# yzhang1918/www2023tiger

Hardware: NVIDIA B200
Metric: events/sec (memory update + embedding, batch 200) (higher is better)
Workload: dtype f32

## Files before the change

include/tiger_b200.h:

```cpp
#ifndef TIGER_B200_H
#define TIGER_B200_H

#include <stdint.h>

#ifdef __cplusplus
extern "C" {
#endif

#define TIGER_OK 0
#define TIGER_EINVAL (-1)
#define TIGER_ECUDA (-2)

#define TIGER_ERR_PAST_MEMORY 1u
#define TIGER_ERR_UNUSED_MSG 2u
#define TIGER_ERR_MSG_BEFORE_MEM 4u
#define TIGER_ERR_MSG_TS_MISMATCH 8u
#define TIGER_ERR_EVENT_BEFORE_MEM 16u
#define TIGER_ERR_CAPACITY 32u

int tiger_abi_version(void);


int64_t tiger_csr_build_work_bytes(int64_t n_events, int64_t n_nodes);
int tiger_csr_build(const int64_t* src, const int64_t* dst, const double* ts, const int64_t* eid,
// ... 9 lines not shown
int tiger_hit_window(const int64_t* center, const int64_t* neigh, int64_t n, int k, float* hit,
                     void* stream);

int tiger_mark_nodes(const int64_t* ids, int64_t n, uint32_t* bitmap, int64_t n_nodes, void* stream);

int tiger_compact_involved(uint32_t* bitmap, int64_t n_nodes, uint8_t* has_msg, uint8_t* uptodate,
                           int64_t* involved, int64_t cap_involved, int64_t* local_index,
                           int64_t* outdated, int32_t* gru_row, int64_t* restart_nodes,
                           int32_t* counts, uint32_t* err_flags, void* stream);


int tiger_select_latest(const int64_t* nids, const void* ts, int ts_is_f64, int64_t n,
                        int64_t ts_period, int64_t n_nodes, uint64_t* slot_ts, uint32_t* slot_pos, uint32_t* bitmap,
                        uint8_t* winner, int64_t* unique_ids, int64_t* index, int32_t* count,
                        void* stream);

int tiger_anonymized_reindex(const int64_t* hist_nids, int64_t n, int len, int64_t* out,
                             const int32_t* count, void* stream);


int tiger_gather_rows(const float* table, int64_t width, const int64_t* ids, int64_t n, float* out,
                      const float* ts_table, float* out_ts, void* stream);

int tiger_scatter_rows(float* table, int64_t width, const int64_t* ids, int64_t n,
                       const int32_t* count, const float* vals, float* ts_table, const float* ts,
                       uint8_t* active, int check, uint32_t* err_flags, void* stream);

int tiger_time_encode(const float* ts, int64_t n, const float* w, const float* b, int dim, float* out,
                      void* stream);

// ... 155 lines not shown
                                  int64_t m_rows, int k_dim, const tiger_left_writeback_fused* wb, void* stream);

int tiger_sgemm_nt_packed_splitk_fused(const float* A, int64_t lda, const float* wpack, int bn, const float* bias,
                                       float* C, int64_t ldc, int k_parts, int64_t m_rows, const int32_t* count,
                                       int64_t rows_per_count, int n_cols, int k_dim, float alpha, int relu,
                                       void* stream);

void* tiger_pipe_create(int n_slots);
void tiger_pipe_destroy(void* pipe);
int tiger_pipe_capture_begin(void* stream);
int tiger_pipe_capture_end(void* pipe, void* stream, int slot, int kind);
int tiger_pipe_submit(void* pipe, int slot, const void* src, void* d_in, int64_t in_bytes, const void* d_out, void* h_out,
                      int64_t out_bytes, void* main_stream);
int tiger_pipe_wait(void* pipe, int slot, int host_results);
int tiger_pipe_join(void* pipe, void* stream);


int tiger_train_gather_pending(const int64_t* ids, const int32_t* count, int64_t cap, const float* msg_vals, int m_dim, const float* msg_ts, const float* upd_vals, int d, const float* check_mem_ts, int check_equal, float* X, float* H, float* dh_zero, uint32_t* err_flags, float* n_rows_out, void* stream);
int tiger_train_gru_gates(const float* Gi, const float* Gh, const float* H, const int32_t* count, int64_t cap, int d, float* h_new, float* r_out, float* z_out, float* n_out, void* stream);
int tiger_train_gru_gates_bwd(const float* dh, const float* r_in, const float* z_in, const float* n_in, const float* Gh, const float* H, const int32_t* count, int64_t cap, int d, float* dGi, float* dGh, void* stream);
int tiger_train_attn_build_ex(const int64_t* center, int64_t n_q, const float* ts, int64_t batch, int64_t ts_group, const int64_t* neigh_nids, const int64_t* neigh_eids, const float* neigh_ts, int k, const float* rows_a, const float* rows_b, const float* key_rows, const int32_t* sel, const float* nfeats, const float* efeats, int d, int de, const float* time_w, const float* time_b, float* q_in, float* kv_in, float* cat, int64_t ld_cat, int cat_off, void* stream);
int tiger_train_attn_core(const float* Q, int64_t ldq, const float* Kp, const float* Vp, int64_t ldkv, const int64_t* neigh_nids, int64_t n_q, int k, int n_head, int head_dim, float p_drop, int seed, float* attn, int64_t ld_attn, float* P, uint32_t* keep_bits, uint8_t* empty, void* stream);
int tiger_train_attn_core_bwd(const float* dattn, int64_t ld_attn, const float* Q, int64_t ldq, const float* Kp, const float* Vp, int64_t ldkv, const float* P, const uint32_t* keep_bits, int64_t n_q, int k, int n_head, int head_dim, float p_drop, float* dQ, float* dKp, float* dVp, void* stream);
int tiger_train_attn_build_bwd_ex(const float* dkv_in, const float* dq_in, const float* dcat, int64_t ld_cat, int cat_off, const int64_t* center, int64_t n_q, const float* ts, int64_t batch, int64_t ts_group, const int64_t* neigh_nids, const float* neigh_ts, int k, const int32_t* sel, int d, int de, const float* time_w, const float* time_b, float* dh_new, float* d_key_rows, float* g_time_w, float* g_time_b, void* stream);
int tiger_train_zero_rows(float* buf, int64_t ld, int cols, int64_t n_rows, const uint8_t* flag, void* stream);
int tiger_train_relu_bwd(float* dy, int64_t ld_dy, const float* y, int64_t ld_y, int cols, int64_t n_rows, const int32_t* count, int64_t rows_per_count, float scale, void* stream);
int tiger_train_colsum(const float* X, int64_t ld, int64_t n_rows, const int32_t* count, int64_t rows_per_count, int cols, float scale, float* out, void* stream);
int tiger_train_scatter_add_rows(float* table, const int64_t* ids, int64_t n, const int32_t* count, int64_t rows_per_count, const float* src, int64_t ld_src, int width, float scale, void* stream);
int tiger_train_score_build(const float* z, const float* hits, const int64_t* neigh_nids, const int64_t* batch_nids, int k, const float* hit_emb, int64_t batch, int d, float* pair, uint8_t* codes, void* stream);
int tiger_train_score_head(float* hid, const float* fc2_w, const float* fc2_b, int64_t batch, int d, float p_drop, int seed, float* scores, float* loss, float* dscore, void* stream);
// ... 27 lines not shown
```

www2023tiger_b200/_lib.py:

```python
import ctypes
import os
import re
from typing import Dict, List

import torch

from .build import INCLUDE, LIB_PATH

P, L, I, F = ctypes.c_void_p, ctypes.c_int64, ctypes.c_int, ctypes.c_float

_SIGNATURES: Dict[str, str] = {
    'tiger_abi_version': '',
    'tiger_csr_build_work_bytes': 'll',
    'tiger_csr_build': 'ppppll' + 'ppppp' + 'p' + 'p',
    'tiger_find_recent': 'ppppp' + 'pp' + 'lli' + 'pppp' + 'pp' + 'p' + 'p',
    'tiger_hit_window': 'ppli' + 'p' + 'p',
    'tiger_mark_nodes': 'plpl' + 'p',
    'tiger_compact_involved': 'plpp' + 'plp' + 'ppp' + 'pp' + 'p',
    'tiger_select_latest': 'ppil' + 'llppp' + 'pppp' + 'p',
    'tiger_anonymized_reindex': 'plip' + 'p' + 'p',
    'tiger_gather_rows': 'plplp' + 'pp' + 'p',
    'tiger_scatter_rows': 'plplp' + 'ppp' + 'pip' + 'p',
    'tiger_time_encode': 'plppip' + 'p',
    'tiger_store_messages': 'ppppl' + 'ppp' + 'ppii' + 'pppp' + 'pp' + 'p',
    'tiger_store_messages_dense': 'ppppl' + 'p' + 'pppp' + 'ppii' + 'pppp' + 'pp' + 'p',
    'tiger_right_writeback': 'plp' + 'ppi' + 'pppp' + 'pppp' + 'p' + 'p',
    'tiger_left_writeback': 'pllp' + 'pip' + 'ppp' + 'p' + 'p',
    'tiger_gru_pack_bytes': 'ii',
    'tiger_gru_pack': 'ppiip' + 'p',
    'tiger_gru_update': 'ppl' + 'plpl' + 'ii' + 'p' + 'ppp' + 'ppi' + 'p' + 'p',
    'tiger_gru_update_rows': 'ppl' + 'plpl' + 'ii' + 'p' + 'ppp' + 'ppi' + 'p' + 'p',
    'tiger_merge_pack': 'piipp',
    'tiger_merge_update': 'ppl' + 'plipl' + 'ii' + 'ppp' + 'ppi' + 'p' + 'p',
    'tiger_attn_fold_bytes': 'iii',
    'tiger_attn_fold': 'piii' + 'p',
    'tiger_temporal_attention_work_bytes': 'liiii',
    'tiger_temporal_attention_ex': 'pplll' + 'pppi' + 'ppppi' + 'pp' + 'iii' + 'ppp' + 'p',
    'tiger_temporal_attention_dense': 'pppppp' + 'li' + 'iii' + 'ppp' + 'p',
    'tiger_score_fold_bytes': 'i',
    'tiger_score_fold_cab_offset': 'i',
    'tiger_score_fold': 'pppppip' + 'p',
    'tiger_link_score_folded': 'pli' + 'pppp' + 'i' + 'ppp' + 'ppp' + 'p',
    'tiger_sgemm_nt_packed_gather': 'ppi' + 'pplp' + 'pi' + 'ppl' + 'lpl' + 'iifi' + 'p',
    'tiger_sgemm_nt_packed_splitk_fused': 'plpi' + 'ppl' + 'i' + 'lpl' + 'iifi' + 'p',
    'tiger_pipe_capture_begin': 'p',
    'tiger_pipe_capture_end': 'ppii',
    'tiger_pipe_submit': 'pipplpplp',
    'tiger_pipe_wait': 'pii',
    'tiger_pipe_join': 'pp',
    'tiger_sgemm_nt_packed_scatter': 'plpippli' + 'pliil' + 'ip' + 'p',
    'tiger_min_time': 'plp' + 'p',
    'tiger_seq_tokens': 'ppli' + 'ppppp' + 'ppii' + 'ppp' + 'ppp' + 'p',
    'tiger_sgemm_nt': 'plplp' + 'pl' + 'lpl' + 'iii' + 'p',
    'tiger_train_gather_pending': 'pplpippipipppppp',
    'tiger_train_gru_gates': 'pppplippppp',
    'tiger_train_gru_gates_bwd': 'ppppppplippp',
    'tiger_train_attn_build_ex': 'plpll' + 'pppi' + 'ppppp' + 'p' + 'ii' + 'pp' + 'ppp' + 'li' + 'p',
    'tiger_train_attn_core': 'plpplpliiifiplpppp',
    'tiger_train_attn_core_bwd': 'plplpplppliiifpppp',
    'tiger_train_attn_build_bwd_ex': 'pppli' + 'plpll' + 'ppi' + 'pii' + 'pp' + 'pppp' + 'p',
    'tiger_train_zero_rows': 'plilpp',
    'tiger_train_relu_bwd': 'plplilplfp',
    'tiger_train_colsum': 'pllplifpp',
    'tiger_train_scatter_add_rows': 'pplplplifp',
# ... 101 lines not shown
```

www2023tiger_b200/csrc/pipe.cu:

```cuda
#include <vector>

#include "common.cuh"

struct TigerPipe {
  int n_slots;
  cudaStream_t s_in, s_out;
  std::vector<cudaGraphExec_t> finder, model, tail;
  std::vector<cudaEvent_t> ev_in, ev_done, ev_out;
  std::vector<char> used, has_out;
  int last_slot;
};

extern "C" void* tiger_pipe_create(int n_slots) {
  if (n_slots <= 0 || n_slots > 1024) return nullptr;
  TigerPipe* p = new TigerPipe();
  p->n_slots = n_slots;
  if (cudaStreamCreateWithFlags(&p->s_in, cudaStreamNonBlocking) != cudaSuccess ||
      cudaStreamCreateWithFlags(&p->s_out, cudaStreamNonBlocking) != cudaSuccess) {
    delete p;
    return nullptr;
  }
  p->finder.assign(n_slots, nullptr);
  p->model.assign(n_slots, nullptr);
  p->tail.assign(n_slots, nullptr);
  p->has_out.assign(n_slots, 0);
  p->last_slot = -1;
  p->ev_in.resize(n_slots);
  p->ev_done.resize(n_slots);
  p->ev_out.resize(n_slots);
  p->used.assign(n_slots, 0);
  for (int i = 0; i < n_slots; ++i) {
    cudaEventCreateWithFlags(&p->ev_in[i], cudaEventDisableTiming);
    cudaEventCreateWithFlags(&p->ev_done[i], cudaEventDisableTiming);
    cudaEventCreateWithFlags(&p->ev_out[i], cudaEventDisableTiming);
  }
  return p;
}

extern "C" void tiger_pipe_destroy(void* pipe) {
  TigerPipe* p = reinterpret_cast<TigerPipe*>(pipe);
  if (p == nullptr) return;
  for (int i = 0; i < p->n_slots; ++i) {
    if (p->finder[i] != nullptr) cudaGraphExecDestroy(p->finder[i]);
    if (p->model[i] != nullptr) cudaGraphExecDestroy(p->model[i]);
    if (p->tail[i] != nullptr) cudaGraphExecDestroy(p->tail[i]);
    cudaEventDestroy(p->ev_in[i]);
    cudaEventDestroy(p->ev_done[i]);
    cudaEventDestroy(p->ev_out[i]);
  }
  cudaStreamDestroy(p->s_in);
  cudaStreamDestroy(p->s_out);
  delete p;
}

extern "C" int tiger_pipe_capture_begin(void* stream) {
  return cudaStreamBeginCapture(as_stream(stream), cudaStreamCaptureModeRelaxed) == cudaSuccess ? TIGER_OK : TIGER_ECUDA;
}

extern "C" int tiger_pipe_capture_end(void* pipe, void* stream, int slot, int kind) {
  TigerPipe* p = reinterpret_cast<TigerPipe*>(pipe);
  cudaGraph_t graph = nullptr;
  if (cudaStreamEndCapture(as_stream(stream), &graph) != cudaSuccess || graph == nullptr) return TIGER_ECUDA;
  if (p == nullptr || slot < 0 || slot >= p->n_slots || kind < 0 || kind > 2) {
    cudaGraphDestroy(graph);
    return TIGER_EINVAL;
  }
  cudaGraphExec_t exec = nullptr;
  const cudaError_t err = cudaGraphInstantiate(&exec, graph, 0);
  cudaGraphDestroy(graph);
  if (err != cudaSuccess) return TIGER_ECUDA;
  cudaGraphExec_t& dst = kind == 0 ? p->finder[slot] : (kind == 1 ? p->model[slot] : p->tail[slot]);
  if (dst != nullptr) cudaGraphExecDestroy(dst);
  dst = exec;
  return TIGER_OK;
}

extern "C" int tiger_pipe_submit(void* pipe, int slot, const void* src, void* d_in, int64_t in_bytes, const void* d_out,
                                 void* h_out, int64_t out_bytes, void* main_stream) {
  TigerPipe* p = reinterpret_cast<TigerPipe*>(pipe);
  if (p == nullptr || slot < 0 || slot >= p->n_slots || p->finder[slot] == nullptr || p->model[slot] == nullptr ||
      src == nullptr || d_in == nullptr || in_bytes <= 0)
    return TIGER_EINVAL;
  cudaStream_t main = as_stream(main_stream);
  bool ok = true;
  if (p->used[slot])
    ok = ok && cudaStreamWaitEvent(p->s_in, p->has_out[slot] ? p->ev_out[slot] : p->ev_done[slot], 0) == cudaSuccess;
  ok = ok && cudaMemcpyAsync(d_in, src, (size_t)in_bytes, cudaMemcpyDefault, p->s_in) == cudaSuccess;
  ok = ok && cudaGraphLaunch(p->finder[slot], p->s_in) == cudaSuccess;
  ok = ok && cudaEventRecord(p->ev_in[slot], p->s_in) == cudaSuccess;
  ok = ok && cudaStreamWaitEvent(main, p->ev_in[slot], 0) == cudaSuccess;
  ok = ok && cudaGraphLaunch(p->model[slot], main) == cudaSuccess;
  ok = ok && cudaEventRecord(p->ev_done[slot], main) == cudaSuccess;
  p->used[slot] = 1;
  p->last_slot = slot;
  const bool download = h_out != nullptr && out_bytes > 0;
  p->has_out[slot] = (p->tail[slot] != nullptr || download) ? 1 : 0;
  if (p->has_out[slot]) {
    ok = ok && cudaStreamWaitEvent(p->s_out, p->ev_done[slot], 0) == cudaSuccess;
    if (p->tail[slot] != nullptr) ok = ok && cudaGraphLaunch(p->tail[slot], p->s_out) == cudaSuccess;
    if (download) ok = ok && cudaMemcpyAsync(h_out, d_out, (size_t)out_bytes, cudaMemcpyDefault, p->s_out) == cudaSuccess;
    ok = ok && cudaEventRecord(p->ev_out[slot], p->s_out) == cudaSuccess;
  }
  return ok ? TIGER_OK : TIGER_ECUDA;
}

extern "C" int tiger_pipe_wait(void* pipe, int slot, int host_results) {
  TigerPipe* p = reinterpret_cast<TigerPipe*>(pipe);
  if (p == nullptr || slot < 0 || slot >= p->n_slots) return TIGER_EINVAL;
  const bool out = host_results && p->has_out[slot];
// ... 10 lines not shown
```

www2023tiger_b200/csrc/select.cu:

```cuda
#include "common.cuh"

#define SELECT_SMALL_N 2048

__device__ __forceinline__ uint64_t load_key(const void* ts, int is_f64, int64_t i) {
  return is_f64 ? orderable_f64(reinterpret_cast<const double*>(ts)[i])
                : orderable_f32(reinterpret_cast<const float*>(ts)[i]);
}

__global__ void __launch_bounds__(1024)
select_latest_small_kernel(const int64_t* __restrict__ nids, const void* __restrict__ ts, int is_f64, int n,
                           int64_t ts_period, uint8_t* __restrict__ winner, int64_t* __restrict__ unique_ids,
                           int64_t* __restrict__ index, int32_t* __restrict__ count) {
  extern __shared__ __align__(16) unsigned char smem_raw[];
  int64_t* s_id = reinterpret_cast<int64_t*>(smem_raw);
  uint64_t* s_key = reinterpret_cast<uint64_t*>(s_id + n);
  uint8_t* s_win = reinterpret_cast<uint8_t*>(s_key + n);
  __shared__ int s_count;
  const int lane = lane_id(), warp = warp_id_in_block(), n_warps = blockDim.x >> 5;
  if (threadIdx.x == 0) s_count = 0;
  for (int p = threadIdx.x; p < n; p += blockDim.x) {
    s_id[p] = nids[p];
    s_key[p] = load_key(ts, is_f64, p % ts_period);
  }
  __syncthreads();
  for (int p = blockIdx.x * n_warps + warp; p < n; p += gridDim.x * n_warps) {
    const int64_t id = s_id[p];
    const uint64_t key = s_key[p];
    bool beaten = false;
    for (int q = lane; q < n; q += 32) {
      if (s_id[q] == id) {
        const uint64_t kq = s_key[q];
        beaten |= (kq > key) || (kq == key && q < p);
      }
// ... 115 lines not shown
                                   int64_t ts_period, int64_t n_nodes, uint64_t* slot_ts, uint32_t* slot_pos, uint32_t* bitmap,
                                   uint8_t* winner, int64_t* unique_ids, int64_t* index, int32_t* count,
                                   void* stream) {
  if (n < 0 || ts_period < 0 || (unique_ids == nullptr) != (index == nullptr)) return TIGER_EINVAL;
  if (ts_period == 0) ts_period = n > 0 ? n : 1;
  cudaStream_t st = as_stream(stream);
  if (n == 0) {
    if (count != nullptr) cudaMemsetAsync(count, 0, sizeof(int32_t), st);
    return tiger_launch_status();
  }
  if (n <= SELECT_SMALL_N) {
    const size_t smem = (size_t)n * (sizeof(int64_t) + sizeof(uint64_t) + 1);
    const bool flags_only = unique_ids == nullptr && count == nullptr;
    const unsigned grid = flags_only ? (unsigned)((n + 31) / 32) : 1u;
    select_latest_small_kernel<<<grid, 1024, smem, st>>>(nids, ts, ts_is_f64, (int)n, ts_period, winner, unique_ids,
                                                        index, count);
    return tiger_launch_status();
  }
  if (slot_ts == nullptr || slot_pos == nullptr || n >= 0xffffffffll) return TIGER_EINVAL;
  if (unique_ids != nullptr && bitmap == nullptr) return TIGER_EINVAL;
  const unsigned grid = (unsigned)((n + 255) / 256);
  select_max_ts_kernel<<<grid, 256, 0, st>>>(nids, ts, ts_is_f64, n, ts_period, slot_ts);
  select_min_pos_kernel<<<grid, 256, 0, st>>>(nids, ts, ts_is_f64, n, ts_period, slot_ts, slot_pos);
  const bool count_in_flags = unique_ids == nullptr && count != nullptr;
  if (count_in_flags) cudaMemsetAsync(count, 0, sizeof(int32_t), st);
  select_flag_kernel<<<grid, 256, 0, st>>>(nids, n, slot_pos, winner, unique_ids != nullptr ? bitmap : nullptr,
                                           count_in_flags ? count : nullptr);
  if (unique_ids != nullptr) {
    select_compact_kernel<<<1, 1024, 0, st>>>(bitmap, (n_nodes + 31) / 32, slot_ts, slot_pos, unique_ids, index,
                                              count);
  } else {
    select_reset_kernel<<<grid, 256, 0, st>>>(nids, n, slot_ts, slot_pos);
  }
  return tiger_launch_status();
}

__global__ void anonymized_reindex_kernel(const int64_t* __restrict__ hist, int len, const int32_t* __restrict__ count,
                                          int64_t* __restrict__ out) {
  extern __shared__ __align__(16) unsigned char smem_raw[];
  int64_t* s_v = reinterpret_cast<int64_t*>(smem_raw);
  uint8_t* s_last = reinterpret_cast<uint8_t*>(s_v + len);
  const int64_t row = blockIdx.x;
  if (count != nullptr && row >= *count) return;
  for (int j = threadIdx.x; j < len; j += blockDim.x) s_v[j] = hist[row * len + j];
  __syncthreads();
  for (int j = threadIdx.x; j < len; j += blockDim.x) {
    bool last = true;
    for (int q = j + 1; q < len; ++q) last = last && (s_v[q] != s_v[j]);
    s_last[j] = last;
  }
  __syncthreads();
// ... 22 lines not shown
```

www2023tiger_b200/engine.py:

```python
from typing import Dict, Optional

import os

import numpy as np
import torch
from torch import Tensor

from . import _lib, ops
from ._lib import raise_on_err_flags
from .ops import f32, f64, i32, i64, u8

KERNELS_PER_STEP = {
    'find_recent': 1, 'compact_involved': 1, 'gru_update': 1, 'temporal_attention': 4, 'select_latest': 1,
    'right_writeback': 1, 'store_messages': 2, 'left_writeback': 0, 'link_score': 1,
}


class TigerEngine:
    def __init__(self, weights: Dict[str, Tensor], csr: ops.DeviceCSR, *, n_nodes: int, dim: int,
                 efeats: Optional[Tensor], nfeats: Optional[Tensor] = None, n_neighbors: int = 10,
                 n_head: int = 2, batch_size: int = 200, msg_src: str = 'left', upd_src: str = 'right',
                 restarter: Optional[str] = None, hist_len: int = 40, hit_type: str = 'bin',
                 lazy_restart: bool = False, want_restarter_targets: bool = False, n_layers: int = 1,
                 msg_tsfm_type: str = 'id', mem_update_type: str = 'gru', device='cuda'):
# ... 18 lines not shown
        self.d = nfeats.shape[1] if nfeats is not None else dim
        self.de = efeats.shape[1] if efeats is not None else dim
        self.M = 3 * self.d + self.de
        self.msg_src, self.upd_src = msg_src, upd_src
        self.restarter, self.hit_type, self.lazy_restart = restarter, hit_type, lazy_restart
        self.want_targets = want_restarter_targets
        N, d, B, K = self.N, self.d, self.B, self.K
        z = lambda *s, dt=f32: torch.zeros(*s, dtype=dt, device=dev)
        self.left_vals, self.left_ts, self.left_active = z(N, d), z(N), z(N, dt=u8)
        self.right_vals, self.right_ts, self.right_active = z(N, d), z(N), z(N, dt=u8)
        self.msg_vals, self.msg_ts, self.has_msg = z(N, self.M), z(N), z(N, dt=u8)
        self.uptodate = z(N, dt=u8)
        self.cap = 3 * B * (K + 1) if n_layers == 1 else min((3 * B + 3 * B * K) * (K + 1), N)
        self.bitmap = z(ops.bitmap_words(N), dt=i32)
        self.involved, self.outdated, self.restart_nodes = z(self.cap, dt=i64), z(self.cap, dt=i64), z(self.cap, dt=i64)
        self.gru_row = torch.full((N,), -1, dtype=i32, device=dev)
        self.counts = z(4, dt=i32)
        self.err_flags = z(1, dt=i32)
        self.neigh_nids, self.neigh_eids = z(3 * B, K, dt=i64), z(3 * B, K, dt=i64)
        self.neigh_ts = z(3 * B, K)
        self.ts32 = z(B)
        if n_layers == 2:
            self.neigh_ts64 = z(3 * B * K, dt=f64)
            self.neigh2_nids, self.neigh2_eids = z(3 * B * K, K, dt=i64), z(3 * B * K, K, dt=i64)
            self.neigh2_ts = z(3 * B * K, K)
            self.emb1 = z(3 * B * K, d)
        self.h_new = z(self.cap, d)
        self.emb = z(3 * B, d)
        self.winner = z(2 * B, dt=u8)
        self.sel_count = z(1, dt=i32)
        self.out_buf = z(2 * B + 1)
        self.hprev_left = z(2 * B, d) if want_restarter_targets else None
        self.hprev_right = z(2 * B, d) if want_restarter_targets else None
        self.inp = z(5 * B, dt=i64)
        self.bind_io(self.inp, self.out_buf)
        self._side = torch.cuda.Stream(device=dev)
        self._serial = int(os.environ.get('TIGER_SERIAL', '0'))
        self._ev_fork, self._ev_side = torch.cuda.Event(), torch.cuda.Event()
        self._ev_fork0, self._ev_rst = torch.cuda.Event(), torch.cuda.Event()
        self.updater = ops.MemoryUpdater(msg_tsfm_type, mem_update_type, self.d, self.M, self.cap, dev)
        self.attn_pack = ops.AttnPack(self.d, self.de, dev, n_head)
        self.attn_pack1 = ops.AttnPack(self.d, self.de, dev, n_head) if n_layers == 2 else None
        self.score_fold = ops.ScoreFold(self.d, dev)
        self.pq = torch.zeros(3 * batch_size, 2 * self.d, dtype=f32, device=dev)
        self.hist_len = hist_len
        self.seq = ops.SeqRestarterOp(self.d, self.de, hist_len, n_head, self.cap, dev) if restarter == 'seq' else None
        self.load_weights(weights)

    def load_weights(self, W: Dict[str, Tensor]):
        g = lambda k: W[k].detach().to(self.device, f32).contiguous()
        self.updater.refresh(g)
        a = 'temporal_embedding_fn.fns.0.'
        self.time_w, self.time_b = g('time_encoder.basis_freq'), g('time_encoder.phase')
        for pack, fa in ((self.attn_pack, a), (self.attn_pack1, 'temporal_embedding_fn.fns.1.')):
            if pack is not None:
                pack.refresh(g(fa + 'mha_fn.q_proj_weight'), g(fa + 'mha_fn.k_proj_weight'),
                             g(fa + 'mha_fn.v_proj_weight'), g(fa + 'mha_fn.in_proj_bias'),
                             g(fa + 'mha_fn.out_proj.weight'), g(fa + 'mha_fn.out_proj.bias'),
                             g(fa + 'merger.fc1.weight'), g(fa + 'merger.fc1.bias'),
                             g(fa + 'merger.fc2.weight'), g(fa + 'merger.fc2.bias'), self.time_w, self.time_b)
        s = 'score_fn.'
        self.score_fold.refresh(g(s + 'fc1.weight'), g(s + 'fc1.bias'), g(s + 'fc2.weight'), g(s + 'fc2.bias'),
                                g(a + 'merger.fc2.weight'), g(a + 'merger.fc2.bias'),
                                g('hit_embedding.weight') if self.hit_type == 'bin' else None)
        self.attn_pack.attach_score_fold(self.score_fold, self.pq)
        if self.restarter == 'static':
            self.left_emb = g('restarter_fn.left_emb.weight')
            self.right_emb = g('restarter_fn.right_emb.weight')
        elif self.restarter == 'seq':
            self.seq.set_weights(W)

    def reset(self):
        for t in (self.left_vals, self.left_ts, self.left_active, self.right_vals, self.right_ts,
                  self.right_active, self.has_msg, self.uptodate, self.err_flags):
            t.zero_()

    def clear_messages(self):
        self.has_msg.zero_()
        self.uptodate.zero_()

    def _mem(self, which):
        if which == 'left':
            return self.left_vals, self.left_ts
        return self.right_vals, self.right_ts

    def check_errors(self):
        raise_on_err_flags(int(self.err_flags.item()) & 0xffffffff)

    def set_batch(self, src, dst, neg, ts, eids):
        B = self.B
        host = torch.empty(5 * B, dtype=i64)
        h = host.numpy()
        h[:B], h[B:2 * B], h[2 * B:3 * B], h[3 * B:4 * B] = src, dst, neg, eids
        h[4 * B:].view(np.float64)[:] = ts
        self.inp.copy_(host)

    def launch_finder(self):
        ops.find_recent(self.csr, self.batch_nids, self.ts64, self.K, ts_period=self.B, want_dirs=False,
                        ts32_out=self.ts32, bitmap=self.bitmap,
                        out=(self.neigh_nids, self.neigh_eids, self.neigh_ts, None))
        if self.n_layers == 2:
            ops.find_second_hop(self.csr, self.neigh_nids, self.neigh_ts, self.K, ts64=self.neigh_ts64,
                                bitmap=self.bitmap, out=(self.neigh2_nids, self.neigh2_eids, self.neigh2_ts))

    def launch_model(self, with_scorer: bool = True):
        d, B = self.d, self.B
        cur = torch.cuda.current_stream()
        serial = self._serial if (torch.cuda.is_current_stream_capturing() or os.environ.get('TIGER_EAGER_BRANCHES') == '1') else 7
        side0 = cur if serial & 1 else self._side
        side1 = cur if serial & 2 else self._side
        msg_vals_mem, msg_ts_mem = self._mem(self.msg_src)
        upd_vals, _ = self._mem(self.upd_src)
        ops.compact_involved(self.bitmap, self.N, self.involved, self.counts, has_msg=self.has_msg,
                             uptodate=self.uptodate if self.lazy_restart else None, outdated=self.outdated,
                             gru_row=self.gru_row, restart_nodes=self.restart_nodes if self.lazy_restart else None,
                             err_flags=self.err_flags)
        main = torch.cuda.current_stream()
        if self.lazy_restart:
            self._ev_fork0.record(main)
            with torch.cuda.stream(side0):
                side0.wait_event(self._ev_fork0)
                if self.restarter == 'static':
                    ops.static_restart(self.restart_nodes, self.cap, self.csr, self.left_emb, self.right_emb, d,
                                       count=self.counts[2:], batch_ts=self.ts32, left_vals=self.left_vals,
                                       left_ts=self.left_ts, left_active=self.left_active, right_vals=self.right_vals,
                                       right_ts=self.right_ts, right_active=self.right_active, has_msg=self.has_msg)
                else:
                    R = self.counts[2:]
                    ops.min_time(self.ts32, self.seq.tmin)
                    self.seq.history(self.csr, self.restart_nodes, self.seq.tmin, self.cap, ts_period=1, count=R)
                    hl, hr, pt = self.seq.forward(self.restart_nodes, self.cap, self.nfeats, self.efeats, count=R)
                    ops.scatter_rows(self.left_vals, self.restart_nodes, hl, ts_table=self.left_ts, ts=pt,
                                     active=self.left_active, count=R)
                    ops.scatter_rows(self.right_vals, self.restart_nodes, hr, ts_table=self.right_ts, ts=pt,
                                     active=self.right_active, count=R)
                self._ev_rst.record(side0)
        self.updater.launch(node_ids=self.outdated, x_table=self.msg_vals, h_table=upd_vals, n_rows=self.cap,
                            out=self.h_new, count=self.counts[1:], msg_ts=self.msg_ts, check_mem_ts=msg_ts_mem,
                            check_equal=(self.msg_src == 'left'), err_flags=self.err_flags)
        if self.lazy_restart and (serial & 2):
            main.wait_event(self._ev_rst)
        self._ev_fork.record(main)
        with torch.cuda.stream(side1):
            side1.wait_event(self._ev_fork)
            ops.select_latest(self.pos, self.ts32, want_unique=False, winner=self.winner, want_count=False)
            ops.right_writeback(self.pos, self.winner, self.gru_row, self.h_new, d, self.right_vals, self.right_ts,
                                self.right_active, self.msg_ts, self.has_msg, self.left_vals, self.hprev_left,
                                self.hprev_right, self.err_flags)
            ops.store_messages(self.src, self.dst, self.eids, self.ts32, self.winner, msg_vals_mem, msg_ts_mem,
                               self.nfeats, self.efeats, d, self.de, self.time_w, self.time_b, self.msg_vals,
                               self.msg_ts, self.has_msg, self.err_flags)
            self._ev_side.record(side1)
        if self.lazy_restart:
            main.wait_event(self._ev_rst)
        key_rows = None
        if self.n_layers == 2:
            ops.temporal_attention(self.attn_pack1, self.H, self.neigh_nids.view(-1), self.ts32, self.neigh2_nids,
                                   self.neigh2_eids, self.neigh2_ts, rows_a=self.right_vals, rows_b=self.h_new,
                                   sel=self.gru_row, nfeats=self.nfeats, efeats=self.efeats, out=self.emb1,
                                   ts_group=self.K)
            key_rows = self.emb1
        self.attn_pack.attach_left_writeback(self.pos, self.winner, self.ts32, self.left_vals, self.left_ts,
                                             self.left_active, self.err_flags, ready_event=self._ev_side)
        ops.temporal_attention(self.attn_pack, self.H, self.batch_nids, self.ts32, self.neigh_nids, self.neigh_eids,
                               self.neigh_ts, rows_a=self.right_vals, rows_b=self.h_new, sel=self.gru_row,
                               nfeats=self.nfeats, efeats=self.efeats, out=self.emb, key_rows=key_rows)
        if with_scorer:
            self.launch_scorer()

    def launch_scorer(self):
        ops.link_score_folded(self.score_fold, self.pq, self.src, self.dst, self.neg,
                              self.neigh_nids if self.hit_type == 'bin' else None, self.scores, self.loss)

    def bind_pq(self, pq: Tensor):
        assert pq.shape == self.pq.shape and pq.dtype == f32
        self.pq = pq
        self.attn_pack.attach_score_fold(self.score_fold, pq)

    def bind_io(self, inp: Tensor, out_buf: Tensor):
        B = self.B
        assert inp.numel() == 5 * B and inp.dtype == i64 and out_buf.numel() == 2 * B + 1 and out_buf.dtype == f32
        self.inp, self.out_buf = inp, out_buf
        self.batch_nids = inp[:3 * B]
        self.src, self.dst, self.neg = inp[:B], inp[B:2 * B], inp[2 * B:3 * B]
        self.pos = inp[:2 * B]
        self.eids = inp[3 * B:4 * B]
        self.ts64 = inp[4 * B:].view(f64)
        self.scores, self.loss = out_buf[:2 * B], out_buf[2 * B:]

    def finder_buffers(self, fresh: bool = False):
        bufs = (self.neigh_nids, self.neigh_eids, self.neigh_ts, self.ts32, self.bitmap)
        if self.n_layers == 2:
            bufs += (self.neigh_ts64, self.neigh2_nids, self.neigh2_eids, self.neigh2_ts)
        if not fresh:
            return bufs
        return tuple(torch.zeros_like(t) for t in bufs)

    def bind_finder(self, bufs):
        self.neigh_nids, self.neigh_eids, self.neigh_ts, self.ts32, self.bitmap = bufs[:5]
        if self.n_layers == 2:
            self.neigh_ts64, self.neigh2_nids, self.neigh2_eids, self.neigh2_ts = bufs[5:]

    def launches_per_step(self) -> int:
        n = sum(KERNELS_PER_STEP.values()) + self.updater.launches - KERNELS_PER_STEP['gru_update']
        if self.n_layers == 2:
            n += 2 + KERNELS_PER_STEP['temporal_attention']
        if self.lazy_restart:
            n += 1 if self.restarter == 'static' else ops.SeqRestarterOp.LAUNCHES + 2
        if self.want_targets:
            n += 1
        return n

    def step(self):
        self.launch_finder()
        self.launch_model()


class StreamRunner:

    def __init__(self, engine: TigerEngine, n_slots: int = 4):
        self.e = engine
        self.graph = None
        self.pipe = None
        B = engine.B
        self.n_slots = n_slots
        self.h_in = [torch.empty(5 * B, dtype=i64).pin_memory() for _ in range(n_slots)]
        self.h_out = [torch.empty(2 * B + 1, dtype=f32).pin_memory() for _ in range(n_slots)]
        self._h_in_np = [t.numpy() for t in self.h_in]
        dev = engine.inp.device
        self.d_in = [torch.zeros(5 * B, dtype=i64, device=dev) for _ in range(n_slots)]
        self.d_out = [torch.zeros(2 * B + 1, dtype=f32, device=dev) for _ in range(n_slots)]
        self.finder_bufs = [engine.finder_buffers(fresh=True) for _ in range(n_slots)]
        self.pq_bufs = [torch.zeros_like(engine.pq) for _ in range(n_slots)]
        self.slot_busy = [False] * n_slots
        self.check_on_wait = False
        self.slot = 0
        self._lib = _lib.load()

    def __del__(self):
        if getattr(self, 'pipe', None):
            self._lib.tiger_pipe_destroy(self.pipe)
            self.pipe = None

    def _check(self, rc: int, what: str):
        if rc != 0:
            raise _lib.TigerLibraryError(f'{what} failed with code {rc}')

    def capture(self, warmup: int = 2):
        e = self.e
        s = torch.cuda.Stream()
        s.wait_stream(torch.cuda.current_stream())
        with torch.cuda.stream(s):
            for _ in range(warmup):
                e.step()
        torch.cuda.current_stream().wait_stream(s)
        torch.cuda.synchronize()
        self.graph = torch.cuda.CUDAGraph()
        with torch.cuda.graph(self.graph):
            e.step()
        torch.cuda.synchronize()
        if self.pipe:
            self._lib.tiger_pipe_destroy(self.pipe)
        self.pipe = self._lib.tiger_pipe_create(self.n_slots)
        if not self.pipe:
            raise _lib.TigerLibraryError('tiger_pipe_create failed')
        inp0, out0, find0, pq0 = e.inp, e.out_buf, e.finder_buffers(), e.pq
        cap = torch.cuda.Stream()
        with torch.cuda.stream(cap):
            for slot in range(self.n_slots):
                e.bind_io(self.d_in[slot], self.d_out[slot])
                e.bind_finder(self.finder_bufs[slot])
                e.bind_pq(self.pq_bufs[slot])
                for kind, launch in ((0, e.launch_finder), (1, lambda: e.launch_model(with_scorer=False)),
                                     (2, e.launch_scorer)):
                    self._check(self._lib.tiger_pipe_capture_begin(cap.cuda_stream), 'capture_begin')
                    try:
                        launch()
                    finally:
                        rc = self._lib.tiger_pipe_capture_end(self.pipe, cap.cuda_stream, slot, kind)
                    self._check(rc, 'capture_end')
        e.bind_io(inp0, out0)
        e.bind_finder(find0)
        e.bind_pq(pq0)
        torch.cuda.synchronize()

    def join(self):
        if self.pipe:
            self._check(self._lib.tiger_pipe_join(self.pipe, _lib.stream_ptr()), 'pipe_join')

    def run_device(self):
        if self.graph is not None:
            self.graph.replay()
        else:
            self.e.step()

    def _next_slot(self) -> int:
        slot = self.slot
        self.slot = (slot + 1) % self.n_slots
        return slot
# ... 55 lines not shown
```

www2023tiger_b200/ops.py:

```python
import ctypes
import os
from typing import Optional, Tuple

import torch
from torch import Tensor

from . import _lib
from ._lib import call, check_cuda, ptr

i64, i32, f32, f64, u8 = torch.int64, torch.int32, torch.float32, torch.float64, torch.uint8


def _empty(shape, dtype, like: Tensor) -> Tensor:
    return torch.empty(shape, dtype=dtype, device=like.device)


class DeviceCSR:

    def __init__(self, indptr, nbr, eid, ts, flag):
        self.indptr, self.nbr, self.eid, self.ts, self.flag = indptr, nbr, eid, ts, flag
        self.n_nodes = indptr.numel() - 1

    @property
    def device(self):
# ... 84 lines not shown
    assert nids.dtype == i64 and ts.dtype in (f32, f64)
    n = nids.numel()
    if winner is None:
        winner = _empty(n, u8, nids)
    uniq = _empty(n, i64, nids) if want_unique else None
    index = _empty(n, i64, nids) if want_unique else None
    if count is None and (want_count or want_unique):
        count = _empty(1, i32, nids)
    if n > 2048 and scratch is None:
        raise _lib.TigerLibraryError('select_latest over more than 2048 positions needs a SelectScratch')
    call('tiger_select_latest', ptr(nids), ptr(ts), int(ts.dtype == f64), n, ts.numel(),
         scratch.n_nodes if scratch else 0, ptr(scratch.slot_ts) if scratch else None,
         ptr(scratch.slot_pos) if scratch else None, ptr(scratch.bitmap) if scratch else None,
         ptr(winner), ptr(uniq), ptr(index), ptr(count))
    return winner, uniq, index, count


def anonymized_reindex(hist_nids: Tensor, out: Optional[Tensor] = None, count: Optional[Tensor] = None) -> Tensor:
    check_cuda(hist_nids)
    n, length = hist_nids.shape
    if out is None:
        out = torch.empty_like(hist_nids)
    call('tiger_anonymized_reindex', ptr(hist_nids), n, length, ptr(out), ptr(count))
    return out


def gather_rows(table: Tensor, ids: Tensor, ts_table: Optional[Tensor] = None):
    check_cuda(table, ids, ts_table)
    n = ids.numel()
    width = table.shape[1]
# ... 572 lines not shown
```

Before: 2.842 million.

## Split model into front/back graphs on separate stream to overlap consecutive steps

Splits the per-step model into a front graph (compact involved nodes, GRU update) that runs on a new front stream, and a back graph (attention, writebacks, messages). The front of the next slot waits only on a side event recorded partway through the previous back graph, not on its whole completion. gru_row and h_new are double-buffered by slot parity so consecutive steps do not overwrite each other. A separate message-timestamp check kernel is folded into the winner-selection kernel. Fence hooks re-serialize the pipeline on reset or weight loads, which adds synchronization complexity and risks data races if the dependencies are wrong.

```diff
diff --git a/include/tiger_b200.h b/include/tiger_b200.h
--- a/include/tiger_b200.h
+++ b/include/tiger_b200.h
@@ -47,6 +47,11 @@
                         int64_t ts_period, int64_t n_nodes, uint64_t* slot_ts, uint32_t* slot_pos, uint32_t* bitmap,
                         uint8_t* winner, int64_t* unique_ids, int64_t* index, int32_t* count,
                         void* stream);
+
+int tiger_select_winners_checked(const int64_t* nids, const float* ts, int64_t n, int64_t ts_period,
+                                 uint8_t* winner, const int64_t* check_ids, const int32_t* check_count,
+                                 const float* msg_ts, const float* mem_ts, int check_equal,
+                                 uint32_t* err_flags, void* stream);
 
 int tiger_anonymized_reindex(const int64_t* hist_nids, int64_t n, int len, int64_t* out,
                              const int32_t* count, void* stream);
@@ -232,6 +237,8 @@
                       int64_t out_bytes, void* main_stream);
 int tiger_pipe_wait(void* pipe, int slot, int host_results);
 int tiger_pipe_join(void* pipe, void* stream);
+int tiger_pipe_capture_mark_side(void* pipe, void* stream, int slot);
+int tiger_pipe_fence(void* pipe);
 
 
 int tiger_train_gather_pending(const int64_t* ids, const int32_t* count, int64_t cap, const float* msg_vals, int m_dim, const float* msg_ts, const float* upd_vals, int d, const float* check_mem_ts, int check_equal, float* X, float* H, float* dh_zero, uint32_t* err_flags, float* n_rows_out, void* stream);
diff --git a/www2023tiger_b200/_lib.py b/www2023tiger_b200/_lib.py
--- a/www2023tiger_b200/_lib.py
+++ b/www2023tiger_b200/_lib.py
@@ -18,6 +18,7 @@
     'tiger_mark_nodes': 'plpl' + 'p',
     'tiger_compact_involved': 'plpp' + 'plp' + 'ppp' + 'pp' + 'p',
     'tiger_select_latest': 'ppil' + 'llppp' + 'pppp' + 'p',
+    'tiger_select_winners_checked': 'ppll' + 'pppp' + 'pip' + 'p',
     'tiger_anonymized_reindex': 'plip' + 'p' + 'p',
     'tiger_gather_rows': 'plplp' + 'pp' + 'p',
     'tiger_scatter_rows': 'plplp' + 'ppp' + 'pip' + 'p',
@@ -48,6 +49,8 @@
     'tiger_pipe_submit': 'pipplpplp',
     'tiger_pipe_wait': 'pii',
     'tiger_pipe_join': 'pp',
+    'tiger_pipe_fence': 'p',
+    'tiger_pipe_capture_mark_side': 'ppi',
     'tiger_sgemm_nt_packed_scatter': 'plpippli' + 'pliil' + 'ip' + 'p',
     'tiger_min_time': 'plp' + 'p',
     'tiger_seq_tokens': 'ppli' + 'ppppp' + 'ppii' + 'ppp' + 'ppp' + 'p',
diff --git a/www2023tiger_b200/csrc/pipe.cu b/www2023tiger_b200/csrc/pipe.cu
--- a/www2023tiger_b200/csrc/pipe.cu
+++ b/www2023tiger_b200/csrc/pipe.cu
@@ -4,11 +4,14 @@
 
 struct TigerPipe {
   int n_slots;
-  cudaStream_t s_in, s_out;
-  std::vector<cudaGraphExec_t> finder, model, tail;
-  std::vector<cudaEvent_t> ev_in, ev_done, ev_out;
+  cudaStream_t s_in, s_out, s_front;
+  std::vector<cudaGraphExec_t> finder, model, tail, front;
+  std::vector<cudaEvent_t> ev_in, ev_done, ev_out, ev_side, ev_front;
+  cudaEvent_t ev_fence;
   std::vector<char> used, has_out;
   int last_slot;
+  cudaStream_t last_main;
+  bool fence;
 };
 
 extern "C" void* tiger_pipe_create(int n_slots) {
@@ -16,24 +19,33 @@
   TigerPipe* p = new TigerPipe();
   p->n_slots = n_slots;
   if (cudaStreamCreateWithFlags(&p->s_in, cudaStreamNonBlocking) != cudaSuccess ||
-      cudaStreamCreateWithFlags(&p->s_out, cudaStreamNonBlocking) != cudaSuccess) {
+      cudaStreamCreateWithFlags(&p->s_out, cudaStreamNonBlocking) != cudaSuccess ||
+      cudaStreamCreateWithFlags(&p->s_front, cudaStreamNonBlocking) != cudaSuccess) {
     delete p;
     return nullptr;
   }
   p->finder.assign(n_slots, nullptr);
   p->model.assign(n_slots, nullptr);
   p->tail.assign(n_slots, nullptr);
+  p->front.assign(n_slots, nullptr);
   p->has_out.assign(n_slots, 0);
   p->last_slot = -1;
+  p->last_main = nullptr;
+  p->fence = true;
   p->ev_in.resize(n_slots);
   p->ev_done.resize(n_slots);
   p->ev_out.resize(n_slots);
+  p->ev_side.resize(n_slots);
+  p->ev_front.resize(n_slots);
   p->used.assign(n_slots, 0);
   for (int i = 0; i < n_slots; ++i) {
     cudaEventCreateWithFlags(&p->ev_in[i], cudaEventDisableTiming);
     cudaEventCreateWithFlags(&p->ev_done[i], cudaEventDisableTiming);
     cudaEventCreateWithFlags(&p->ev_out[i], cudaEventDisableTiming);
+    cudaEventCreateWithFlags(&p->ev_side[i], cudaEventDisableTiming);
+    cudaEventCreateWithFlags(&p->ev_front[i], cudaEventDisableTiming);
   }
+  cudaEventCreateWithFlags(&p->ev_fence, cudaEventDisableTiming);
   return p;
 }
 
@@ -44,12 +56,17 @@
     if (p->finder[i] != nullptr) cudaGraphExecDestroy(p->finder[i]);
     if (p->model[i] != nullptr) cudaGraphExecDestroy(p->model[i]);
     if (p->tail[i] != nullptr) cudaGraphExecDestroy(p->tail[i]);
+    if (p->front[i] != nullptr) cudaGraphExecDestroy(p->front[i]);
     cudaEventDestroy(p->ev_in[i]);
     cudaEventDestroy(p->ev_done[i]);
     cudaEventDestroy(p->ev_out[i]);
+    cudaEventDestroy(p->ev_side[i]);
+    cudaEventDestroy(p->ev_front[i]);
   }
+  cudaEventDestroy(p->ev_fence);
   cudaStreamDestroy(p->s_in);
   cudaStreamDestroy(p->s_out);
+  cudaStreamDestroy(p->s_front);
   delete p;
 }
 
@@ -61,7 +78,7 @@
   TigerPipe* p = reinterpret_cast<TigerPipe*>(pipe);
   cudaGraph_t graph = nullptr;
   if (cudaStreamEndCapture(as_stream(stream), &graph) != cudaSuccess || graph == nullptr) return TIGER_ECUDA;
-  if (p == nullptr || slot < 0 || slot >= p->n_slots || kind < 0 || kind > 2) {
+  if (p == nullptr || slot < 0 || slot >= p->n_slots || kind < 0 || kind > 3) {
     cudaGraphDestroy(graph);
     return TIGER_EINVAL;
   }
@@ -69,9 +86,24 @@
   const cudaError_t err = cudaGraphInstantiate(&exec, graph, 0);
   cudaGraphDestroy(graph);
   if (err != cudaSuccess) return TIGER_ECUDA;
-  cudaGraphExec_t& dst = kind == 0 ? p->finder[slot] : (kind == 1 ? p->model[slot] : p->tail[slot]);
+  std::vector<cudaGraphExec_t>* kinds[] = {&p->finder, &p->model, &p->tail, &p->front};
+  cudaGraphExec_t& dst = (*kinds[kind])[slot];
   if (dst != nullptr) cudaGraphExecDestroy(dst);
   dst = exec;
+  return TIGER_OK;
+}
+
+extern "C" int tiger_pipe_capture_mark_side(void* pipe, void* stream, int slot) {
+  TigerPipe* p = reinterpret_cast<TigerPipe*>(pipe);
+  if (p == nullptr || slot < 0 || slot >= p->n_slots) return TIGER_EINVAL;
+  return cudaEventRecordWithFlags(p->ev_side[slot], as_stream(stream), cudaEventRecordExternal) == cudaSuccess
+             ? TIGER_OK : TIGER_ECUDA;
+}
+
+extern "C" int tiger_pipe_fence(void* pipe) {
+  TigerPipe* p = reinterpret_cast<TigerPipe*>(pipe);
+  if (p == nullptr) return TIGER_EINVAL;
+  p->fence = true;
   return TIGER_OK;
 }
 
@@ -79,7 +111,7 @@
                                  void* h_out, int64_t out_bytes, void* main_stream) {
   TigerPipe* p = reinterpret_cast<TigerPipe*>(pipe);
   if (p == nullptr || slot < 0 || slot >= p->n_slots || p->finder[slot] == nullptr || p->model[slot] == nullptr ||
-      src == nullptr || d_in == nullptr || in_bytes <= 0)
+      p->front[slot] == nullptr || src == nullptr || d_in == nullptr || in_bytes <= 0)
     return TIGER_EINVAL;
   cudaStream_t main = as_stream(main_stream);
   bool ok = true;
@@ -88,11 +120,24 @@
   ok = ok && cudaMemcpyAsync(d_in, src, (size_t)in_bytes, cudaMemcpyDefault, p->s_in) == cudaSuccess;
   ok = ok && cudaGraphLaunch(p->finder[slot], p->s_in) == cudaSuccess;
   ok = ok && cudaEventRecord(p->ev_in[slot], p->s_in) == cudaSuccess;
-  ok = ok && cudaStreamWaitEvent(main, p->ev_in[slot], 0) == cudaSuccess;
+  const int prev = p->last_slot;
+  if (prev >= 0 && p->last_main != main) ok = ok && cudaStreamWaitEvent(main, p->ev_done[prev], 0) == cudaSuccess;
+  if (p->fence || prev < 0) {
+    ok = ok && cudaEventRecord(p->ev_fence, main) == cudaSuccess;
+    ok = ok && cudaStreamWaitEvent(p->s_front, p->ev_fence, 0) == cudaSuccess;
+    p->fence = false;
+  } else {
+    ok = ok && cudaStreamWaitEvent(p->s_front, p->ev_side[prev], 0) == cudaSuccess;
+  }
+  ok = ok && cudaStreamWaitEvent(p->s_front, p->ev_in[slot], 0) == cudaSuccess;
+  ok = ok && cudaGraphLaunch(p->front[slot], p->s_front) == cudaSuccess;
+  ok = ok && cudaEventRecord(p->ev_front[slot], p->s_front) == cudaSuccess;
+  ok = ok && cudaStreamWaitEvent(main, p->ev_front[slot], 0) == cudaSuccess;
   ok = ok && cudaGraphLaunch(p->model[slot], main) == cudaSuccess;
   ok = ok && cudaEventRecord(p->ev_done[slot], main) == cudaSuccess;
   p->used[slot] = 1;
   p->last_slot = slot;
+  p->last_main = main;
   const bool download = h_out != nullptr && out_bytes > 0;
   p->has_out[slot] = (p->tail[slot] != nullptr || download) ? 1 : 0;
   if (p->has_out[slot]) {
diff --git a/www2023tiger_b200/csrc/select.cu b/www2023tiger_b200/csrc/select.cu
--- a/www2023tiger_b200/csrc/select.cu
+++ b/www2023tiger_b200/csrc/select.cu
@@ -1,6 +1,25 @@
 #include "common.cuh"
 
 #define SELECT_SMALL_N 2048
+
+struct MsgTsCheck {
+  const int64_t* ids;
+  const int32_t* count;
+  const float* msg_ts;
+  const float* mem_ts;
+  int check_equal;
+  uint32_t* err_flags;
+};
+
+__device__ __forceinline__ void msg_ts_check(const MsgTsCheck& c) {
+  const int n = *c.count;
+  for (int j = blockIdx.x * blockDim.x + threadIdx.x; j < n; j += gridDim.x * blockDim.x) {
+    const int64_t u = c.ids[j];
+    const float mt = c.msg_ts[u], pt = c.mem_ts[u];
+    if (pt > mt) atomicOr(c.err_flags, TIGER_ERR_MSG_BEFORE_MEM);
+    if (c.check_equal && mt != pt) atomicOr(c.err_flags, TIGER_ERR_MSG_TS_MISMATCH);
+  }
+}
 
 __device__ __forceinline__ uint64_t load_key(const void* ts, int is_f64, int64_t i) {
   return is_f64 ? orderable_f64(reinterpret_cast<const double*>(ts)[i])
@@ -10,13 +29,15 @@
 __global__ void __launch_bounds__(1024)
 select_latest_small_kernel(const int64_t* __restrict__ nids, const void* __restrict__ ts, int is_f64, int n,
                            int64_t ts_period, uint8_t* __restrict__ winner, int64_t* __restrict__ unique_ids,
-                           int64_t* __restrict__ index, int32_t* __restrict__ count) {
+                           int64_t* __restrict__ index, int32_t* __restrict__ count,
+                           const MsgTsCheck chk) {
   extern __shared__ __align__(16) unsigned char smem_raw[];
   int64_t* s_id = reinterpret_cast<int64_t*>(smem_raw);
   uint64_t* s_key = reinterpret_cast<uint64_t*>(s_id + n);
   uint8_t* s_win = reinterpret_cast<uint8_t*>(s_key + n);
   __shared__ int s_count;
   const int lane = lane_id(), warp = warp_id_in_block(), n_warps = blockDim.x >> 5;
+  if (chk.ids != nullptr) msg_ts_check(chk);
   if (threadIdx.x == 0) s_count = 0;
   for (int p = threadIdx.x; p < n; p += blockDim.x) {
     s_id[p] = nids[p];
@@ -162,7 +183,7 @@
     const bool flags_only = unique_ids == nullptr && count == nullptr;
     const unsigned grid = flags_only ? (unsigned)((n + 31) / 32) : 1u;
     select_latest_small_kernel<<<grid, 1024, smem, st>>>(nids, ts, ts_is_f64, (int)n, ts_period, winner, unique_ids,
-                                                        index, count);
+                                                        index, count, MsgTsCheck{});
     return tiger_launch_status();
   }
   if (slot_ts == nullptr || slot_pos == nullptr || n >= 0xffffffffll) return TIGER_EINVAL;
@@ -183,6 +204,21 @@
   return tiger_launch_status();
 }
 
+extern "C" int tiger_select_winners_checked(const int64_t* nids, const float* ts, int64_t n, int64_t ts_period,
+                                            uint8_t* winner, const int64_t* check_ids, const int32_t* check_count,
+                                            const float* msg_ts, const float* mem_ts, int check_equal,
+                                            uint32_t* err_flags, void* stream) {
+  if (n <= 0 || n > SELECT_SMALL_N || ts_period < 0 || winner == nullptr || check_ids == nullptr ||
+      check_count == nullptr || msg_ts == nullptr || mem_ts == nullptr || err_flags == nullptr)
+    return TIGER_EINVAL;
+  if (ts_period == 0) ts_period = n;
+  const size_t smem = (size_t)n * (sizeof(int64_t) + sizeof(uint64_t) + 1);
+  const MsgTsCheck chk{check_ids, check_count, msg_ts, mem_ts, check_equal, err_flags};
+  select_latest_small_kernel<<<(unsigned)((n + 31) / 32), 1024, smem, as_stream(stream)>>>(
+      nids, ts, 0, (int)n, ts_period, winner, nullptr, nullptr, nullptr, chk);
+  return tiger_launch_status();
+}
+
 __global__ void anonymized_reindex_kernel(const int64_t* __restrict__ hist, int len, const int32_t* __restrict__ count,
                                           int64_t* __restrict__ out) {
   extern __shared__ __align__(16) unsigned char smem_raw[];
diff --git a/www2023tiger_b200/engine.py b/www2023tiger_b200/engine.py
--- a/www2023tiger_b200/engine.py
+++ b/www2023tiger_b200/engine.py
@@ -1,6 +1,7 @@
-from typing import Dict, Optional
+from typing import Dict, NamedTuple, Optional
 
 import os
+import weakref
 
 import numpy as np
 import torch
@@ -56,7 +57,10 @@
         self.cap = 3 * B * (K + 1) if n_layers == 1 else min((3 * B + 3 * B * K) * (K + 1), N)
         self.bitmap = z(ops.bitmap_words(N), dt=i32)
         self.involved, self.outdated, self.restart_nodes = z(self.cap, dt=i64), z(self.cap, dt=i64), z(self.cap, dt=i64)
-        self.gru_row = torch.full((N,), -1, dtype=i32, device=dev)
+        self.gru_rows = [torch.full((N,), -1, dtype=i32, device=dev) for _ in range(2)]
+        self.h_news = [z(self.cap, d) for _ in range(2)]
+        self.gru_row, self.h_new = self.gru_rows[0], self.h_news[0]
+        self._n_steps = 0
         self.counts = z(4, dt=i32)
         self.err_flags = z(1, dt=i32)
         self.neigh_nids, self.neigh_eids = z(3 * B, K, dt=i64), z(3 * B, K, dt=i64)
@@ -67,7 +71,6 @@
             self.neigh2_nids, self.neigh2_eids = z(3 * B * K, K, dt=i64), z(3 * B * K, K, dt=i64)
             self.neigh2_ts = z(3 * B * K, K)
             self.emb1 = z(3 * B * K, d)
-        self.h_new = z(self.cap, d)
         self.emb = z(3 * B, d)
         self.winner = z(2 * B, dt=u8)
         self.sel_count = z(1, dt=i32)
@@ -77,6 +80,7 @@
         self.inp = z(5 * B, dt=i64)
         self.bind_io(self.inp, self.out_buf)
         self._side = torch.cuda.Stream(device=dev)
+        self._fence_hooks = []
         self._serial = int(os.environ.get('TIGER_SERIAL', '0'))
         self._ev_fork, self._ev_side = torch.cuda.Event(), torch.cuda.Event()
         self._ev_fork0, self._ev_rst = torch.cuda.Event(), torch.cuda.Event()
@@ -90,6 +94,7 @@
         self.load_weights(weights)
 
     def load_weights(self, W: Dict[str, Tensor]):
+        self._fence()
         g = lambda k: W[k].detach().to(self.device, f32).contiguous()
         self.updater.refresh(g)
         a = 'temporal_embedding_fn.fns.0.'
@@ -113,13 +118,27 @@
             self.seq.set_weights(W)
 
     def reset(self):
+        self._fence()
         for t in (self.left_vals, self.left_ts, self.left_active, self.right_vals, self.right_ts,
-                  self.right_active, self.has_msg, self.uptodate, self.err_flags):
+                  self.right_active, self.has_msg, self.uptodate, self.err_flags, *self.h_news):
             t.zero_()
+        self._n_steps = 0
 
     def clear_messages(self):
+        self._fence()
         self.has_msg.zero_()
         self.uptodate.zero_()
+
+    def add_fence_hook(self, fn):
+        self._fence_hooks.append(weakref.WeakMethod(fn))
+
+    def _fence(self):
+        for ref in list(self._fence_hooks):
+            fn = ref()
+            if fn is None:
+                self._fence_hooks.remove(ref)
+            else:
+                fn()
 
     def _mem(self, which):
         if which == 'left':
@@ -145,21 +164,24 @@
             ops.find_second_hop(self.csr, self.neigh_nids, self.neigh_ts, self.K, ts64=self.neigh_ts64,
                                 bitmap=self.bitmap, out=(self.neigh2_nids, self.neigh2_eids, self.neigh2_ts))
 
-    def launch_model(self, with_scorer: bool = True):
-        d, B = self.d, self.B
+    def _branches(self) -> int:
+        if torch.cuda.is_current_stream_capturing() or os.environ.get('TIGER_EAGER_BRANCHES') == '1':
+            return self._serial
+        return 7
+
+    def launch_front(self, bufs: Optional['SlotBuffers'] = None):
+        if bufs is not None:
+            self.bind(bufs)
+        d = self.d
         cur = torch.cuda.current_stream()
-        serial = self._serial if (torch.cuda.is_current_stream_capturing() or os.environ.get('TIGER_EAGER_BRANCHES') == '1') else 7
-        side0 = cur if serial & 1 else self._side
-        side1 = cur if serial & 2 else self._side
-        msg_vals_mem, msg_ts_mem = self._mem(self.msg_src)
+        side0 = cur if self._branches() & 1 else self._side
         upd_vals, _ = self._mem(self.upd_src)
         ops.compact_involved(self.bitmap, self.N, self.involved, self.counts, has_msg=self.has_msg,
                              uptodate=self.uptodate if self.lazy_restart else None, outdated=self.outdated,
                              gru_row=self.gru_row, restart_nodes=self.restart_nodes if self.lazy_restart else None,
                              err_flags=self.err_flags)
-        main = torch.cuda.current_stream()
         if self.lazy_restart:
-            self._ev_fork0.record(main)
+            self._ev_fork0.record(cur)
             with torch.cuda.stream(side0):
                 side0.wait_event(self._ev_fork0)
                 if self.restarter == 'static':
@@ -178,23 +200,33 @@
                                      active=self.right_active, count=R)
                 self._ev_rst.record(side0)
         self.updater.launch(node_ids=self.outdated, x_table=self.msg_vals, h_table=upd_vals, n_rows=self.cap,
-                            out=self.h_new, count=self.counts[1:], msg_ts=self.msg_ts, check_mem_ts=msg_ts_mem,
-                            check_equal=(self.msg_src == 'left'), err_flags=self.err_flags)
-        if self.lazy_restart and (serial & 2):
-            main.wait_event(self._ev_rst)
+                            out=self.h_new, count=self.counts[1:], msg_ts=self.msg_ts, check_mem_ts=None,
+                            check_equal=False, err_flags=self.err_flags)
+        if self.lazy_restart:
+            cur.wait_event(self._ev_rst)
+
+    def launch_back(self, bufs: Optional['SlotBuffers'] = None, with_scorer: bool = True, mark_side=None):
+        if bufs is not None:
+            self.bind(bufs)
+        d = self.d
+        main = torch.cuda.current_stream()
+        side1 = main if self._branches() & 2 else self._side
+        msg_vals_mem, msg_ts_mem = self._mem(self.msg_src)
         self._ev_fork.record(main)
         with torch.cuda.stream(side1):
             side1.wait_event(self._ev_fork)
-            ops.select_latest(self.pos, self.ts32, want_unique=False, winner=self.winner, want_count=False)
+            ops.select_winners_checked(self.pos, self.ts32, self.winner, check_ids=self.outdated,
+                                       check_count=self.counts[1:], msg_ts=self.msg_ts, mem_ts=msg_ts_mem,
+                                       check_equal=(self.msg_src == 'left'), err_flags=self.err_flags)
             ops.right_writeback(self.pos, self.winner, self.gru_row, self.h_new, d, self.right_vals, self.right_ts,
                                 self.right_active, self.msg_ts, self.has_msg, self.left_vals, self.hprev_left,
                                 self.hprev_right, self.err_flags)
             ops.store_messages(self.src, self.dst, self.eids, self.ts32, self.winner, msg_vals_mem, msg_ts_mem,
                                self.nfeats, self.efeats, d, self.de, self.time_w, self.time_b, self.msg_vals,
                                self.msg_ts, self.has_msg, self.err_flags)
+            if mark_side is not None and self.upd_src == 'right':
+                mark_side()
             self._ev_side.record(side1)
-        if self.lazy_restart:
-            main.wait_event(self._ev_rst)
         key_rows = None
         if self.n_layers == 2:
             ops.temporal_attention(self.attn_pack1, self.H, self.neigh_nids.view(-1), self.ts32, self.neigh2_nids,
@@ -207,6 +239,9 @@
         ops.temporal_attention(self.attn_pack, self.H, self.batch_nids, self.ts32, self.neigh_nids, self.neigh_eids,
                                self.neigh_ts, rows_a=self.right_vals, rows_b=self.h_new, sel=self.gru_row,
                                nfeats=self.nfeats, efeats=self.efeats, out=self.emb, key_rows=key_rows)
+        if mark_side is not None and self.upd_src == 'left':
+            main.wait_event(self._ev_side)
+            mark_side()
         if with_scorer:
             self.launch_scorer()
 
@@ -230,18 +265,28 @@
         self.ts64 = inp[4 * B:].view(f64)
         self.scores, self.loss = out_buf[:2 * B], out_buf[2 * B:]
 
-    def finder_buffers(self, fresh: bool = False):
+    def finder_buffers(self, fresh: bool = False, half: Optional[int] = None):
         bufs = (self.neigh_nids, self.neigh_eids, self.neigh_ts, self.ts32, self.bitmap)
         if self.n_layers == 2:
             bufs += (self.neigh_ts64, self.neigh2_nids, self.neigh2_eids, self.neigh2_ts)
-        if not fresh:
-            return bufs
-        return tuple(torch.zeros_like(t) for t in bufs)
+        if fresh:
+            bufs = tuple(torch.zeros_like(t) for t in bufs)
+        ring = (self.gru_row, self.h_new) if half is None else (self.gru_rows[half], self.h_news[half])
+        return bufs + ring
 
     def bind_finder(self, bufs):
         self.neigh_nids, self.neigh_eids, self.neigh_ts, self.ts32, self.bitmap = bufs[:5]
         if self.n_layers == 2:
-            self.neigh_ts64, self.neigh2_nids, self.neigh2_eids, self.neigh2_ts = bufs[5:]
+            self.neigh_ts64, self.neigh2_nids, self.neigh2_eids, self.neigh2_ts = bufs[5:9]
+        self.gru_row, self.h_new = bufs[-2:]
+
+    def slot_buffers(self) -> 'SlotBuffers':
+        return SlotBuffers(self.inp, self.out_buf, self.finder_buffers(), self.pq)
+
+    def bind(self, bufs: 'SlotBuffers'):
+        self.bind_io(bufs.inp, bufs.out_buf)
+        self.bind_finder(bufs.finder)
+        self.bind_pq(bufs.pq)
 
     def launches_per_step(self) -> int:
         n = sum(KERNELS_PER_STEP.values()) + self.updater.launches - KERNELS_PER_STEP['gru_update']
@@ -254,13 +299,28 @@
         return n
 
     def step(self):
+        self._fence()
+        half = self._n_steps % 2
+        self._n_steps += 1
+        self.gru_row, self.h_new = self.gru_rows[half], self.h_news[half]
         self.launch_finder()
-        self.launch_model()
+        self.launch_front()
+        self.launch_back()
+
+
+class SlotBuffers(NamedTuple):
+    inp: Tensor
+    out_buf: Tensor
+    finder: tuple
+    pq: Tensor
 
 
 class StreamRunner:
 
     def __init__(self, engine: TigerEngine, n_slots: int = 4):
+        if n_slots < 2 or n_slots % 2:
+            raise ValueError(f'n_slots={n_slots}: the gru_row / h_new ring is indexed by slot parity, use an even '
+                             f'number of at least 2')
         self.e = engine
         self.graph = None
         self.pipe = None
@@ -272,11 +332,14 @@
         dev = engine.inp.device
         self.d_in = [torch.zeros(5 * B, dtype=i64, device=dev) for _ in range(n_slots)]
         self.d_out = [torch.zeros(2 * B + 1, dtype=f32, device=dev) for _ in range(n_slots)]
-        self.finder_bufs = [engine.finder_buffers(fresh=True) for _ in range(n_slots)]
+        self.finder_bufs = [engine.finder_buffers(fresh=True, half=slot % 2) for slot in range(n_slots)]
         self.pq_bufs = [torch.zeros_like(engine.pq) for _ in range(n_slots)]
+        self.slot_bufs = [SlotBuffers(self.d_in[s], self.d_out[s], self.finder_bufs[s], self.pq_bufs[s])
+                          for s in range(n_slots)]
         self.slot_busy = [False] * n_slots
         self.check_on_wait = False
         self.slot = 0
+        self._hooked = False
         self._lib = _lib.load()
 
     def __del__(self):
@@ -306,25 +369,31 @@
         self.pipe = self._lib.tiger_pipe_create(self.n_slots)
         if not self.pipe:
             raise _lib.TigerLibraryError('tiger_pipe_create failed')
-        inp0, out0, find0, pq0 = e.inp, e.out_buf, e.finder_buffers(), e.pq
+        bound = e.slot_buffers()
         cap = torch.cuda.Stream()
         with torch.cuda.stream(cap):
             for slot in range(self.n_slots):
-                e.bind_io(self.d_in[slot], self.d_out[slot])
-                e.bind_finder(self.finder_bufs[slot])
-                e.bind_pq(self.pq_bufs[slot])
-                for kind, launch in ((0, e.launch_finder), (1, lambda: e.launch_model(with_scorer=False)),
+                mark = lambda: self._check(self._lib.tiger_pipe_capture_mark_side(
+                    self.pipe, torch.cuda.current_stream().cuda_stream, slot), 'capture_mark_side')
+                for kind, launch in ((0, e.launch_finder), (3, e.launch_front),
+                                     (1, lambda: e.launch_back(with_scorer=False, mark_side=mark)),
                                      (2, e.launch_scorer)):
+                    e.bind(self.slot_bufs[slot])
                     self._check(self._lib.tiger_pipe_capture_begin(cap.cuda_stream), 'capture_begin')
                     try:
                         launch()
                     finally:
                         rc = self._lib.tiger_pipe_capture_end(self.pipe, cap.cuda_stream, slot, kind)
                     self._check(rc, 'capture_end')
-        e.bind_io(inp0, out0)
-        e.bind_finder(find0)
-        e.bind_pq(pq0)
+        e.bind(bound)
         torch.cuda.synchronize()
+        if not self._hooked:
+            e.add_fence_hook(self.fence)
+            self._hooked = True
+
+    def fence(self):
+        if self.pipe:
+            self._check(self._lib.tiger_pipe_fence(self.pipe), 'pipe_fence')
 
     def join(self):
         if self.pipe:
diff --git a/www2023tiger_b200/ops.py b/www2023tiger_b200/ops.py
--- a/www2023tiger_b200/ops.py
+++ b/www2023tiger_b200/ops.py
@@ -122,6 +122,14 @@
          ptr(scratch.slot_pos) if scratch else None, ptr(scratch.bitmap) if scratch else None,
          ptr(winner), ptr(uniq), ptr(index), ptr(count))
     return winner, uniq, index, count
+
+
+def select_winners_checked(nids: Tensor, ts: Tensor, winner: Tensor, *, check_ids: Tensor, check_count: Tensor,
+                           msg_ts: Tensor, mem_ts: Tensor, check_equal: bool, err_flags: Tensor):
+    check_cuda(nids, ts, winner, check_ids, check_count, msg_ts, mem_ts, err_flags)
+    assert nids.dtype == i64 and ts.dtype == f32 and winner.dtype == u8
+    call('tiger_select_winners_checked', ptr(nids), ptr(ts), nids.numel(), ts.numel(), ptr(winner), ptr(check_ids),
+         ptr(check_count), ptr(msg_ts), ptr(mem_ts), int(check_equal), ptr(err_flags))
 
 
 def anonymized_reindex(hist_nids: Tensor, out: Optional[Tensor] = None, count: Optional[Tensor] = None) -> Tensor:
```

Result: faster. 2.977 million, median of 6 (+4.8%).
